# shuwang127/SRCNN_Cpp

Measured on AMD Instinct MI355X. Metric: SRCNN Y-channel Mpixels/sec, higher is better.
Workload: dtype f32; 1 GPU; 1 x 3840x2160 luma plane per GPU per step (1920x1080 x2.0, BASELINE configs[1]), fused conv path, mfma arithmetic, inputs resident in HBM; frames_per_gpu=1, width=3840, height=2160, mode=mfma, seam_deferral=True, output_checksum=584152

## Files before the change

srcnn_cpp_amd/csrc/srcnn_kernels.h:

```cpp
#pragma once
#include <hip/hip_runtime.h>
#include <stddef.h>
#include <stdint.h>

namespace srcnn {

constexpr int FW = 128;
constexpr int YP = FW + 8;
constexpr int YR = 16;
constexpr int NWAVES = FW / 32;
constexpr int NTHREADS = NWAVES * 64;

enum StripMode { MODE_FUSED = 0, MODE_L12 = 1, MODE_L3 = 2 };

constexpr int NFRAG_L1 = 82;
constexpr int NFRAG_L2 = 32;
constexpr int NFRAG_L3 = 16;
constexpr int NFRAG_B2 = 16;
constexpr int NFRAG_L2U = 32;
constexpr int NFRAG_B2U = 16;
constexpr int NFRAG_L3U = 16;
constexpr int FRAG_L2 = NFRAG_L1, FRAG_L3 = FRAG_L2 + NFRAG_L2, FRAG_B2 = FRAG_L3 + NFRAG_L3,
              FRAG_L2U = FRAG_B2 + NFRAG_B2, FRAG_B2U = FRAG_L2U + NFRAG_L2U, FRAG_L3U = FRAG_B2U + NFRAG_B2U;
constexpr int NFRAG = FRAG_L3U + NFRAG_L3U;

__host__ __device__ constexpr int acc_row(int r, int h) { return (r & 3) + 8 * (r >> 2) + 4 * h; }
__host__ __device__ constexpr int row_chan(int i) { return 2 * ((i & 3) + 4 * (i >> 3)) + ((i >> 2) & 1); }

__host__ __device__ constexpr int l3_row_tap(int i)
{
    const int r = (i & 3) + 4 * (i >> 3), h = (i >> 2) & 1, s = r / 5, m = r % 5, n = h ? 3 + s : s;
    return (r < 15 && n < 5) ? 5 * m + n : -1;
}
__host__ __device__ constexpr bool l3_row_is_scale(int i)
{
    const int r = (i & 3) + 4 * (i >> 3), h = (i >> 2) & 1;
    return h == 1 && r >= 10 && r < 15;
}

constexpr int S16_FRAG_L2 = 24, S16_FRAG_L3 = 32, S16_NFRAG = 36;
constexpr size_t S16_TABLE_BYTES = (size_t)S16_NFRAG * 64 * 16 + 2 * 16 * sizeof(float);
__host__ __device__ constexpr int l1s_tap(int b, int h, int e)
{
    const int n = 4 * b + e / 2, u = e & 1;
    if (n < 20) return (2 * (n % 5) + u < 9) ? 9 * (n / 5 + 5 * h) + 2 * (n % 5) + u : -1;
    if (n < 23) {
        const int jj = 4 * h + 2 * (n - 20) + u;
        return (h == 0 ? jj <= 3 : (jj >= 4 && jj <= 8)) ? 36 + jj : -1;
    }
    return (u == 0 && h == 0) ? 81 : -1;
}

struct StripParams {
    const uint8_t *src;
    long src_stride, src_frame_pitch;
    int src_row0;
    const uint8_t *src_top, *src_bot;
    long halo_stride;
    int src_row1;
    const float *planes_in;
    float *planes_out;
    long pl_stride, pl_pitch, pl_frame_pitch;
    uint8_t *dst;
    float *pre;
    long dst_stride, dst_frame_pitch;
    int dst_row0;
    const float *wfrag;
    const uint32_t *wfrag16;
    float *sink;
    float b3;
    int width, height;
    int row_begin, row_end;
    int seg_rows, n_strips, n_segs;
    const int *items;
    int items_per_frame;
    int seams_per_frame;
    float *seam;
    float *cseam;
    int strips_total;
    int tune;
    uint8_t *flag;
    float fix_delta, fix_scale;
    float fix_kl, fix_abs;
    unsigned *fix_counters;
};

enum { FIX_N_SCAT = 0, FIX_N_DENSE = 1, FIX_N_CHANGED = 2, FIX_MAX_DEV = 3, FIX_N_RERUN = 4,
       FIX_MAX_RATIO = 5,
       FIX_TOTALS = 6,
       FIX_WORD_STRIDE = 64,
       FIX_NEXT_ITEM = 6,
       FIX_NEXT_RERUN = 7,
       FIX_REGIONS = 8, FIX_REGION0 = 8 * FIX_WORD_STRIDE,
       FIX_COUNTERS = FIX_REGION0 + FIX_REGIONS * FIX_WORD_STRIDE };
struct FixParams {
    const uint8_t *src;
    long src_stride;
    int src_row0;
    const uint8_t *src_top, *src_bot;
    long halo_stride;
    int src_row1;
    uint8_t *dst;
    const uint8_t *flag;
    long dst_stride;
    int dst_row0;
    int width, height, row_begin, row_end;
    const float *wraw;
    unsigned *counters;
    unsigned long long *totals;
    unsigned *scat, *dense;
// ... 106 lines not shown
```

srcnn_cpp_amd/csrc/srcnn_mfma.hip:

```cpp
#include "srcnn_kernels.h"

#include <type_traits>

#ifndef SRCNN_SAFE_HAZARDS
#define SRCNN_SAFE_HAZARDS 0
#endif
#if SRCNN_SAFE_HAZARDS
#define SRCNN_KNS safe
#else
#define SRCNN_KNS fast
#endif

namespace srcnn {
namespace SRCNN_KNS {

typedef float f32x16 __attribute__((ext_vector_type(16)));
typedef float f32x2 __attribute__((ext_vector_type(2)));

#define MFMA(a, b, c) __builtin_amdgcn_mfma_f32_32x32x2f32((a), (b), (c), 0, 0, 0)

__device__ __forceinline__ f32x16 mfma_first(float a, float b, const f32x16 &c)
{
#if SRCNN_SAFE_HAZARDS
    return MFMA(a, b, c);
#endif
    f32x16 d;
    asm volatile("v_mfma_f32_32x32x2_f32 %0, %1, %2, %3" : "=&v"(d) : "v"(a), "v"(b), "v"(c));
    return d;
}
__device__ __forceinline__ f32x16 mfma_first0(float a, float b)
{
#if SRCNN_SAFE_HAZARDS
    const f32x16 z = {0};
    return MFMA(a, b, z);
#endif
    f32x16 d;
    asm volatile("v_mfma_f32_32x32x2_f32 %0, %1, %2, 0" : "=&v"(d) : "v"(a), "v"(b));
    return d;
}


__device__ __forceinline__ int clampi(int v, int lo, int hi) { return min(max(v, lo), hi); }

__device__ __forceinline__ unsigned lane_off(unsigned x)
{
    asm volatile("" : "+v"(x));
    return x;
}
template <typename T>
__device__ __forceinline__ __attribute__((address_space(1))) T *scalar_base(T *p)
{
    __attribute__((address_space(1))) T *g = (__attribute__((address_space(1))) T *)p;
    asm volatile("" : "+s"(g));
    return g;
}

template <typename T>
__device__ __forceinline__ T *uniform_ptr(T *p)
{
    const unsigned long long a = (unsigned long long)p;
    const unsigned lo = __builtin_amdgcn_readfirstlane((unsigned)a), hi = __builtin_amdgcn_readfirstlane((unsigned)(a >> 32));
    return (T *)(((unsigned long long)hi << 32) | lo);
}

__device__ __forceinline__ void lds_barrier()
{
    asm volatile("s_waitcnt lgkmcnt(0)\n\ts_barrier" ::: "memory");
}

__device__ __forceinline__ float relu(float x)
{
    float r;
    asm("v_max_f32 %0, 0, %1" : "=v"(r) : "v"(x));
    return r;
}

__device__ const signed char CSEAM_TERMS[15][9] = {
    {4, 0, 124, 1, 125, 2, 126, 3, 127}, {3, 0, 125, 1, 126, 2, 127, 0, 0}, {1, 0, 126, 0, 0, 0, 0, 0, 0},
    {1, 0, 127, 0, 0, 0, 0, 0, 0},       {1, 1, 127, 0, 0, 0, 0, 0, 0},     {1, 2, 0, 0, 0, 0, 0, 0, 0},
    {1, 3, 1, 0, 0, 0, 0, 0, 0},         {1, 4, 2, 0, 0, 0, 0, 0, 0},       {1, 1, 0, 0, 0, 0, 0, 0, 0},
    {1, 2, 1, 0, 0, 0, 0, 0, 0},         {1, 3, 2, 0, 0, 0, 0, 0, 0},       {1, 4, 3, 0, 0, 0, 0, 0, 0},
    {1, 3, 0, 0, 0, 0, 0, 0, 0},         {1, 4, 0, 0, 0, 0, 0, 0, 0},       {1, 4, 1, 0, 0, 0, 0, 0, 0}};

struct CseamLane {
    int cnt, off[4];
};
__device__ __forceinline__ CseamLane cseam_lane(int e)
{
    CseamLane cl = {0, {0, 0, 0, 0}};
    if (e < 15) {
        const signed char *t = CSEAM_TERMS[e];
        cl.cnt = t[0];
#pragma unroll
        for (int i = 0; i < 4; ++i) cl.off[i] = i < t[0] ? t[1 + 2 * i] * FW + t[2 + 2 * i] : 0;
    }
    return cl;
}
__device__ __forceinline__ void cseam_export(const float *tile, float *dst, int e, const CseamLane &cl)
{
    const float a = tile[cl.off[0]], b = tile[cl.off[1]], c = tile[cl.off[2]], d = tile[cl.off[3]];
    float v = a;
    v = cl.cnt > 1 ? v + b : v;
    v = cl.cnt > 2 ? v + c : v;
    v = cl.cnt > 3 ? v + d : v;
    if (cl.cnt > 0) dst[(unsigned)e] = v;
}

__device__ __forceinline__ void relu_pairs(f32x16 &a, const f32x2 ones)
{
#if SRCNN_SAFE_HAZARDS
#pragma unroll
    for (int q = 0; q < 16; ++q) a[q] = __builtin_fmaxf(a[q], 0.f);
    return;
#endif
#pragma unroll
    for (int q = 0; q < 8; ++q) {
        f32x2 pr = {a[2 * q], a[2 * q + 1]};
        asm("v_pk_mul_f32 %0, %0, %1 clamp" : "+v"(pr) : "s"(ones));
        a[2 * q] = pr.x;
        a[2 * q + 1] = pr.y;
    }
}

constexpr bool fast_kernel(int mode, bool pre, int diag)
{
    (void)diag;
    return mode == MODE_FUSED && !pre;
}

template <int MODE, bool PRE, int DIAG = 0, bool FIX = false, bool HALO3 = false>
__device__ __forceinline__ void strip_body(const StripParams &p)
{
    static_assert(!FIX || (MODE == MODE_FUSED && !PRE && DIAG == 0), "flags belong to the production fused kernel");
    static_assert(!HALO3 || (MODE == MODE_FUSED && !PRE && DIAG == 0), "halo buffers belong to the production fused kernel");
    if constexpr (FIX) {
        if (blockIdx.x == 0)
            for (int i = threadIdx.x; i < FIX_COUNTERS; i += 256) p.fix_counters[i] = 0u;
    }
    unsigned long long lt[4] = {0, 0, 0, 0};
    if constexpr (DIAG == 2) lt[0] = __builtin_amdgcn_s_memrealtime();
    extern __shared__ __attribute__((aligned(16))) char smem[];
    float *ylds = reinterpret_cast<float *>(smem);
    float *fbuf = (MODE == MODE_L3) ? ylds : ylds + 2 * YR * YP;

    const int tid = threadIdx.x;
    const int lane = tid & 63;
    const int wave = __builtin_amdgcn_readfirstlane(tid >> 6);
    const int j = lane & 31;
    const int half = lane >> 5;

    constexpr int HALO = (MODE == MODE_L12) ? 0 : 2;

    const int W = p.width, H = p.height;
    int bid = blockIdx.x;
    int strip, frame = 0, ys, ye, seam_up = -1, seam_dn = -1;
    if (p.items) {
        frame = bid / p.items_per_frame;
        const int *it = p.items + ITEM_INTS * (bid - frame * p.items_per_frame);
        strip = it[0];
        ys = it[1];
        ye = it[2];
        if constexpr (MODE == MODE_FUSED) {
            seam_up = it[3] >= 0 ? it[3] + frame * p.seams_per_frame : -1;
            seam_dn = it[4] >= 0 ? it[4] + frame * p.seams_per_frame : -1;
        }
        if (ys >= ye) return;
    } else {
        if (!(p.tune & 8)) {
            const int nwg = gridDim.x, q = nwg >> 3, r = nwg & 7, xcd = bid & 7;
            bid = (xcd < r ? xcd * (q + 1) : r * (q + 1) + (xcd - r) * q) + (bid >> 3);
        }
        strip = bid % p.n_strips;
        bid /= p.n_strips;
        const int seg = bid % p.n_segs;
        frame = bid / p.n_segs;
        ys = p.row_begin + seg * p.seg_rows;
        ye = min(ys + p.seg_rows, p.row_end);
    }

    const bool cs = (MODE != MODE_L12) && p.cseam != nullptr;
    const CseamLane cl = cseam_lane((cs && threadIdx.x < 64 && (threadIdx.x & 31) < 15 &&
                                     (threadIdx.x < 32 || fast_kernel(MODE, PRE, DIAG)))
                                        ? (int)(threadIdx.x & 31) : 15);
    const int halo_c = cs ? 0 : HALO;
    const int xs = strip * (FW - 2 * halo_c);
    const int gx0 = xs - halo_c;
    float *cs_row0 = (cs && wave == 0)
                         ? p.cseam + (((long)frame * p.strips_total + strip) * (p.row_end - p.row_begin) - p.row_begin) * CSEAM_FLOATS
                         : nullptr;
    const bool top_open = seam_up >= 0, bot_open = seam_dn >= 0;
    const int f_lo = top_open ? ys : max(ys - HALO, 0);
    const int f_hi = bot_open ? ye : min(ye + HALO, H);
    const int out_lo = top_open ? ys + 2 : ys, out_hi = bot_open ? ye - 2 : ye;

    const float *wf = p.wfrag + lane;
    float w1f[2][41], w2f[32], w3f[16];
    f32x16 b2v = {0};
    if constexpr (MODE != MODE_L3) {
#pragma unroll
        for (int t = 0; t < 2; ++t)
#pragma unroll
            for (int s = 0; s < 41; ++s) w1f[t][s] = wf[(t * 41 + s) * 64];
        constexpr int L2 = (MODE == MODE_L12) ? FRAG_L2U : FRAG_L2, B2 = (MODE == MODE_L12) ? FRAG_B2U : FRAG_B2;
#pragma unroll
        for (int q = 0; q < 32; ++q) w2f[q] = wf[(L2 + q) * 64];
#pragma unroll
        for (int q = 0; q < 16; ++q) b2v[q] = wf[(B2 + q) * 64];
    }
    if constexpr (MODE != MODE_L12) {
        constexpr int L3 = (MODE == MODE_L3) ? FRAG_L3U : FRAG_L3;
#pragma unroll
        for (int q = 0; q < 16; ++q) w3f[q] = wf[(L3 + q) * 64];
    }
    const f32x2 ones = {1.0f, 1.0f};

    const uint8_t *srcf = nullptr;
    int ycol = 0;
    if constexpr (MODE != MODE_L3) {
        srcf = p.src + (long)frame * p.src_frame_pitch;
        ycol = clampi(gx0 - 4 + tid, 0, W - 1);
    }
    const int y_last = min(H - 1, f_hi + 3);
    auto y_row = [&](int r) -> const uint8_t * {
        if constexpr (HALO3) {
            if (r < p.src_row0) return p.src_top + (long)(r - (p.src_row0 - 6)) * p.halo_stride;
            if (r >= p.src_row1) return p.src_bot + (long)(r - p.src_row1) * p.halo_stride;
        }
        return srcf + (long)(r - p.src_row0) * p.src_stride;
    };
    auto load_y = [&](int r) -> uint8_t {
        const uint8_t *row = y_row(clampi(r, 0, y_last));
        return row[(unsigned)ycol];
    };
    auto stage_y = [&](int r, uint8_t v) {
        const int slot = r & (YR - 1);
        const float fv = (float)v;
        ylds[slot * YP + tid] = fv;
        ylds[(slot + YR) * YP + tid] = fv;
    };
    if constexpr (MODE != MODE_L3) {
        if (tid < YP) {
            uint8_t v[9];
#pragma unroll
            for (int q = 0; q < 9; ++q) v[q] = load_y(f_lo - 4 + q);
#pragma unroll
            for (int q = 0; q < 9; ++q) stage_y(f_lo - 4 + q, v[q]);
        }
        __syncthreads();
    }
    asm volatile("s_waitcnt vmcnt(0)" ::: "memory");
    if constexpr (MODE != MODE_L3) {
#pragma unroll
        for (int t = 0; t < 2; ++t)
#pragma unroll
            for (int k = 0; k < 41; ++k) asm volatile("" : "+v"(w1f[t][k]));
#pragma unroll
        for (int q = 0; q < 32; ++q) asm volatile("" : "+v"(w2f[q]));
        asm volatile("" : "+v"(b2v));
    }
    if constexpr (MODE != MODE_L12) {
#pragma unroll
        for (int q = 0; q < 16; ++q) asm volatile("" : "+v"(w3f[q]));
    }

    if constexpr (DIAG == 2) lt[1] = __builtin_amdgcn_s_memrealtime();

    const int xi = 32 * wave + j;
    const int gx = gx0 + xi;


    constexpr bool FASTK = fast_kernel(MODE, PRE, DIAG);
    static_assert(!FIX || FASTK, "the flag threshold reads plane 5 through the FAST kernels' column offsets");
    constexpr int FSLOT = 6 * FW;
    int xn[5] = {0, 0, 0, 0, 0};
    bool px_ok = false;
    if constexpr (MODE != MODE_L12) {
#pragma unroll
        for (int n = 0; n < 5; ++n) {
            xn[n] = clampi(clampi(gx + n - 2, 0, W - 1) - gx0, 0, FW - 1);
            if constexpr (FASTK) xn[n] += n * FW + half * FSLOT;
        }
        px_ok = cs ? (gx < W) && (xi >= 2 || strip == 0) && (xi < FW - 2 || strip == p.strips_total - 1)
                   : (xi >= HALO) && (xi < FW - HALO) && (gx < W);
    }
    CseamLane cl2 = cl;
    if constexpr (FASTK) {
#pragma unroll
        for (int i = 0; i < 4; ++i) cl2.off[i] += half * FSLOT;
    }
    float R[4][3] = {{0.f, 0.f, 0.f}, {0.f, 0.f, 0.f}, {0.f, 0.f, 0.f}, {0.f, 0.f, 0.f}};
    long o_out = (long)frame * p.dst_frame_pitch + (long)(f_lo - 3 - p.dst_row0) * p.dst_stride;
    long o_src = (long)(min(f_lo + 5, y_last) - p.src_row0) * p.src_stride;
    long o_pl = (long)frame * p.pl_frame_pitch + (long)(MODE == MODE_L3 ? min(f_lo + 1, H - 1) : f_lo) * p.pl_stride;
    auto scale_thr = [&](const float *fr) -> float {
        float s1 = fr[xn[0] + 5 * FW];
#pragma unroll
        for (int n = 1; n < 5; ++n) s1 += fr[xn[n] + (5 - n) * FW];
        return fix_threshold(s1, p.fix_delta, p.fix_kl, p.fix_abs);
    };
    auto finalize = [&](long o, float acc, bool ok, const float *fr) {
        const float v = acc + p.b3;
        auto row = scalar_base(p.dst + o);
        if (ok) row[lane_off((unsigned)gx)] = (uint8_t)clampi((int)v, 0, 255);
        if constexpr (FIX) {
            auto frow = scalar_base(p.flag + o);
            const float thr = scale_thr(fr);
            if (ok) frow[lane_off((unsigned)gx)] = fix_code(v, thr, p.fix_delta, p.fix_scale);
        }
        if constexpr (PRE) {
            float *prow = p.pre + o;
            if (ok) prow[(unsigned)gx] = v;
        }
    };
    auto ftile = [&](int g, int slot) -> float * {
        if constexpr (FASTK) return fbuf + ((4 - ((g + slot) & 3)) & 3) * FSLOT;
        else return fbuf + (((g & 1) * 3 + slot) * 6) * FW;
    };
    auto vertical = [&](int f, const f32x16 &t) {
        const int fplane = 3 * half * FW + xi;
        if (top_open && f < ys + SEAM_ROWS) {
            const int r = f - ys;
            float *o = p.seam + ((long)seam_up * SEAM_FLOATS + seam_t_off(r)) * NTHREADS + tid;
#pragma unroll
            for (int s = 0; s < 3; ++s)
#pragma unroll
                for (int m = 1; m < 5; ++m)
                    if (m > r) o[(s * (4 - r) + (m - r - 1)) * NTHREADS] = t[5 * s + m];
        }
        if (f > 0) {
            float *fo = ftile(f, 0) + fplane;
#pragma unroll
            for (int s = 0; s < 3; ++s) {
                fo[s * FW] = R[3][s] + t[5 * s + 4];
                R[3][s] = R[2][s] + t[5 * s + 3];
                R[2][s] = R[1][s] + t[5 * s + 2];
                R[1][s] = R[0][s] + t[5 * s + 1];
                R[0][s] = t[5 * s];
            }
        } else {
#pragma unroll
            for (int s = 0; s < 3; ++s) {
                R[0][s] = t[5 * s];
                R[1][s] = t[5 * s] + t[5 * s + 1];
                R[2][s] = R[1][s] + t[5 * s + 2];
                R[3][s] = 0.f;
            }
        }
        if (f == H - 1) {
            float *f1 = ftile(f, 1) + fplane, *f2 = ftile(f, 2) + fplane;
#pragma unroll
            for (int s = 0; s < 3; ++s) {
                f1[s * FW] = R[3][s] + t[5 * s + 4];
                f2[s * FW] = (R[2][s] + t[5 * s + 3]) + t[5 * s + 4];
            }
        }
    };
    float hv[5];
    auto hp_load = [&](int g, int slot) {
        const float *fr = ftile(g, slot);
#pragma unroll
        for (int n = 0; n < 5; ++n) hv[n] = FASTK ? fr[xn[n]] : fr[n * FW + xn[n]];
    };
    auto hp_use = [&](int g, int slot) {
        float acc = hv[0];
#pragma unroll
        for (int n = 1; n < 5; ++n) acc += hv[n];
        const int y = g - 2 + slot;
        const bool rows_ok = (y >= out_lo) && (y < out_hi) && (!FASTK || half == 0);
        finalize(slot == 0 ? o_out : o_out + (long)slot * p.dst_stride, acc, px_ok && rows_ok, ftile(g, slot));
        if (cs_row0 && rows_ok) cseam_export(ftile(g, slot), cs_row0 + y * CSEAM_FLOATS, lane, FASTK ? cl2 : cl);
    };
    const unsigned st2 = (unsigned)gx + (half ? 0u : (unsigned)p.dst_stride);
    const unsigned cs2 = (unsigned)(lane & 31) + (half ? 0u : (unsigned)CSEAM_FLOATS);
    const int do_cs = __builtin_amdgcn_readfirstlane((cs && wave == 0) ? 1 : 0);
    auto hp2_load = [&](int slot) {
        const float *fr = fbuf + slot * FSLOT;
#pragma unroll
        for (int n = 0; n < 5; ++n) hv[n] = fr[xn[n]];
    };
    float v2 = 0.f;
    auto hp2_use = [&](int f, int slot) {
        float acc = hv[0];
#pragma unroll
        for (int n = 1; n < 5; ++n) acc += hv[n];
        const float v = acc + p.b3;
        auto row = scalar_base(p.dst + (o_out - p.dst_stride));
        if (px_ok) row[lane_off(st2)] = (uint8_t)clampi((int)v, 0, 255);
        if constexpr (FIX) {
            v2 = v;
            const float *fr = fbuf + slot * FSLOT;
#pragma unroll
            for (int n = 0; n < 5; ++n) hv[n] = fr[xn[n] + (5 - n) * FW];
        }
        if (do_cs) {
            const float *tile = fbuf + slot * FSLOT;
            const float a = tile[cl2.off[0]], b = tile[cl2.off[1]], c = tile[cl2.off[2]], d = tile[cl2.off[3]];
            float e = a;
            e = cl2.cnt > 1 ? e + b : e;
            e = cl2.cnt > 2 ? e + c : e;
            e = cl2.cnt > 3 ? e + d : e;
            auto dst = scalar_base(cs_row0 + (f - 4) * CSEAM_FLOATS);
            if (cl2.cnt > 0) dst[cs2] = e;
        }
    };

    auto hp2_flag = [&]() {
        float s1 = hv[0];
#pragma unroll
        for (int n = 1; n < 5; ++n) s1 += hv[n];
        const float thr = fix_threshold(s1, p.fix_delta, p.fix_kl, p.fix_abs);
        auto frow = scalar_base(p.flag + (o_out - p.dst_stride));
        if (px_ok) frow[lane_off(st2)] = fix_code(v2, thr, p.fix_delta, p.fix_scale);
    };

    f32x16 d2n = {0};
    const unsigned pl_lane = (MODE == MODE_L12) ? (unsigned)(half * p.pl_pitch + gx)
                                                : (unsigned)(half * p.pl_pitch + clampi(gx, 0, W - 1));
    auto load_planes_at = [&](long o) {
        const float *q = p.planes_in + o;
        const unsigned lo = lane_off(pl_lane * 4u);
#pragma unroll
        for (int r = 0; r < 16; ++r)
            d2n[r] = __builtin_nontemporal_load((const __attribute__((address_space(1))) float *)((const __attribute__((address_space(1))) char *)scalar_base(q + (long)(2 * r) * p.pl_pitch) + lo));
    };
    if constexpr (MODE == MODE_L3) load_planes_at((long)frame * p.pl_frame_pitch + (long)f_lo * p.pl_stride);
    auto drain = [&](int g) {
        const int nslots = (g == H - 1) ? 3 : 1;
        for (int slot = 0; slot < nslots; ++slot) {
            hp_load(g, slot);
            hp_use(g, slot);
        }
    };
    auto row = [&](int f, auto ph_tag) {
        constexpr int PH = decltype(ph_tag)::value;
        constexpr bool FAST = PH >= 0;
        const int g = f - 1;
        const bool hp = FAST ? (PH & 1) != 0 : (MODE != MODE_L12) && (g >= f_lo);
        constexpr int SLOT_W = (4 - PH) & 3;
        constexpr int SLOT_R = (4 - ((PH + 3) & 3)) & 3;

        f32x16 d2;
        if constexpr (MODE != MODE_L3) {
            unsigned ynext;
            asm volatile("" : "=v"(ynext));
            if constexpr (HALO3) {
                const uint8_t *yr = uniform_ptr(y_row(min(f + 5, y_last)));
                if (tid < YP) ynext = scalar_base(yr)[lane_off((unsigned)ycol)];
            } else {
                if (tid < YP) ynext = scalar_base(srcf + o_src)[lane_off((unsigned)ycol)];
                if (f + 5 < y_last) o_src += p.src_stride;
            }

            const float *yb = ylds + ((f - 4) & (YR - 1)) * YP + xi;
            const float *ybN = yb + half;
            const float *ybW = yb + (half ? YP - 8 : 0);
            auto ldb = [&](int s) -> float {
                const int ki = (2 * s) / 9, kj = (2 * s) % 9;
                if (s == 40) return half ? 1.0f : yb[8 * YP + 8];
                if (kj == 8) return ybW[ki * YP + kj];
                return ybN[ki * YP + kj];
            };
            f32x16 a0 = {0}, a1 = {0};
            auto layer1 = [&](auto with_pb) {
                constexpr bool PB = decltype(with_pb)::value;
                constexpr int PF = 3;
                float bq[41];
#pragma unroll
                for (int s = 0; s < PF; ++s) bq[s] = ldb(s);
#pragma unroll
                for (int s = 0; s < 41; ++s) {
                    if (s + PF < 41) bq[s + PF] = ldb(s + PF);
                    if constexpr (PB && MODE != MODE_L12) {
                        if constexpr (FAST) {
                            if (s == 2) hp2_load(SLOT_R);
                            if (s == 8) hp2_use(f, SLOT_R);
                            if constexpr (FIX) {
                                if (s == 14) hp2_flag();
                            }
                        } else {
                            if (s == 2) hp_load(g, 0);
                            if (s == 8) hp_use(g, 0);
                        }
                    }
                    a0 = MFMA(w1f[0][s], bq[s], a0);
                    a1 = MFMA(w1f[1][s], bq[s], a1);
                    __builtin_amdgcn_sched_barrier(0);
                }
            };
            if constexpr (FAST) {
                layer1(std::integral_constant<bool, (PH & 1) != 0>{});
            } else {
                if (hp) layer1(std::true_type{});
                else layer1(std::false_type{});
            }
            relu_pairs(a0, ones);
            relu_pairs(a1, ones);
            __builtin_amdgcn_sched_barrier(0);

            d2 = mfma_first(w2f[0], a0[0], b2v);
#pragma unroll
            for (int r = 1; r < 16; ++r) d2 = MFMA(w2f[r], a0[r], d2);
#pragma unroll
            for (int r = 0; r < 16; ++r) d2 = MFMA(w2f[16 + r], a1[r], d2);
            __builtin_amdgcn_sched_barrier(0);
            if constexpr (MODE == MODE_L12) {
#pragma unroll
                for (int r = 0; r < 16; ++r) d2[r] = relu(d2[r]);
            } else {
                relu_pairs(d2, ones);
            }
            __builtin_amdgcn_sched_barrier(0);

            asm volatile("" : "+v"(ynext));
            if (tid < YP) stage_y(f + 5, (uint8_t)ynext);

            if constexpr (MODE == MODE_L12) {
                if (gx < W) {
                    float *o = p.planes_out + o_pl;
                    const unsigned lo = lane_off(pl_lane * 4u);
#pragma unroll
                    for (int r = 0; r < 16; ++r)
                        __builtin_nontemporal_store(d2[r], (__attribute__((address_space(1))) float *)((__attribute__((address_space(1))) char *)scalar_base(o + (long)(2 * r) * p.pl_pitch) + lo));
                }
            }
        } else {
            d2 = d2n;
            load_planes_at(o_pl);
            if constexpr (FAST) {
                if constexpr ((PH & 1) != 0) {
                    hp2_load(SLOT_R);
                    hp2_use(f, SLOT_R);
                }
            } else if (hp) {
                hp_load(g, 0);
                hp_use(g, 0);
            }
        }

        if constexpr (MODE != MODE_L12) {
            f32x16 t = {0};
            if constexpr (MODE == MODE_FUSED) {
                t = mfma_first0(w3f[0], d2[0]);
#pragma unroll
                for (int r = 1; r < 16; ++r) t = MFMA(w3f[r], d2[r], t);
            } else {
#pragma unroll
                for (int r = 0; r < 16; ++r) t = MFMA(w3f[r], d2[r], t);
            }
            __builtin_amdgcn_sched_barrier(0);
            if constexpr (FAST) {
                float *fo = fbuf + SLOT_W * FSLOT + 3 * half * FW + xi;
#pragma unroll
                for (int s = 0; s < 3; ++s) {
                    fo[s * FW] = R[3][s] + t[5 * s + 4];
#ifndef SRCNN_ABL_NO_CHAIN_ADDS
                    R[3][s] = R[2][s] + t[5 * s + 3];
                    R[2][s] = R[1][s] + t[5 * s + 2];
                    R[1][s] = R[0][s] + t[5 * s + 1];
                    R[0][s] = t[5 * s];
#endif
                    asm volatile("" : "+v"(R[0][s]), "+v"(R[1][s]), "+v"(R[2][s]), "+v"(R[3][s]));
                }
            } else {
                vertical(f, t);
            }
        }

        if constexpr (FASTK) __builtin_amdgcn_sched_barrier(0);
        lds_barrier();
        if constexpr (FASTK) __builtin_amdgcn_sched_barrier(0);
        o_out += p.dst_stride;
        if constexpr (MODE == MODE_L3) {
            if (f + 1 < H - 1) o_pl += p.pl_stride;
        } else {
            o_pl += p.pl_stride;
        }
    };
    {
        int f = f_lo;
        if constexpr (FASTK) {
            const int f_a = (f_lo + 6 + 1) & ~1;
            const int f_b = min(f_hi, H - 1) & ~1;
            for (; f < f_hi && f < f_a; ++f) row(f, std::integral_constant<int, -1>{});
            if ((f & 2) && f + 2 <= f_b) {
                row(f, std::integral_constant<int, 2>{});
                row(f + 1, std::integral_constant<int, 3>{});
// ... 177 lines not shown
    if (winmap && (winmap[(long)v * rows + yrel] | winmap[(long)(v + 1) * rows + yrel])) return;
    const float *es = p.cseam + (((long)frame * p.strips_total + v) * rows + yrel) * CSEAM_FLOATS;
    const float *et = es + (long)rows * CSEAM_FLOATS;
    cseam_pixels<PRE, FIX>(p, es, et, frame, p.row_begin + yrel, (v + 1) * FW);
}

template <bool PRE, bool FIX>
__global__ __launch_bounds__(256) void srcnn_cseam_kernel(const StripParams p)
{
    cseam_block<PRE, FIX>(p, (long)blockIdx.x, (int)blockIdx.y, nullptr);
}

template <bool PRE, bool FIX>
__global__ __launch_bounds__(NTHREADS) void srcnn_seams_merged_kernel(const StripParams p, const int *__restrict__ seams, int n_seams,
                                                                     const unsigned char *__restrict__ winmap, int cblocks_per_frame)
{
    static_assert(NTHREADS == 256, "both roles use 256 threads");
    if ((int)blockIdx.x < n_seams) {
        seam_block<PRE, true, FIX>(p, seams, (int)blockIdx.x);
    } else {
        const int q = (int)blockIdx.x - n_seams;
        cseam_block<PRE, FIX>(p, (long)(q % cblocks_per_frame), q / cblocks_per_frame, winmap);
    }
}

size_t strip_lds_bytes(int mode);

template <bool HALO3>
__global__ __launch_bounds__(NTHREADS, 2) void srcnn_strip_fold_kernel(const StripParams p, const FoldParams f)
{
    if ((int)blockIdx.x >= f.first_block) {
        const int q = (int)blockIdx.x - f.first_block;
        if (q >= f.n_seams) cseam_block<false, false>(f.prev, (long)(q - f.n_seams), 0, f.winmap);
        else if (f.winmap) seam_block<false, true, false>(f.prev, f.seams, q);
        else seam_block<false, false, false>(f.prev, f.seams, q);
        return;
    }
    fast::strip_body<MODE_FUSED, false, 0, false, HALO3>(p);
}

hipError_t launch_strip_fold(const StripParams &p, const FoldParams &f, hipStream_t stream, size_t lds_pad)
{
    if (p.pre || p.flag || f.prev.pre || f.prev.flag || !p.items) return hipErrorInvalidValue;
    const dim3 grid((unsigned)(f.first_block + f.n_seams + f.cblocks)), block(NTHREADS);
    const size_t lds = strip_lds_bytes(MODE_FUSED) + lds_pad;
    if (p.src_top || p.src_bot) hipLaunchKernelGGL((srcnn_strip_fold_kernel<true>), grid, block, lds, stream, p, f);
    else hipLaunchKernelGGL((srcnn_strip_fold_kernel<false>), grid, block, lds, stream, p, f);
    return hipGetLastError();
}

hipError_t launch_cseams(const StripParams &p, int n_frames, hipStream_t stream)
{
    const long n = (long)(p.strips_total - 1) * (p.row_end - p.row_begin);
    if (n <= 0) return hipSuccess;
    const dim3 grid((unsigned)((n + 255) / 256), (unsigned)n_frames);
    if (p.flag) hipLaunchKernelGGL((srcnn_cseam_kernel<false, true>), grid, dim3(256), 0, stream, p);
    else if (p.pre) hipLaunchKernelGGL((srcnn_cseam_kernel<true, false>), grid, dim3(256), 0, stream, p);
    else hipLaunchKernelGGL((srcnn_cseam_kernel<false, false>), grid, dim3(256), 0, stream, p);
    return hipGetLastError();
}

hipError_t launch_seams_merged(const StripParams &p, int n_seams , const int *d_seams, const unsigned char *d_winmap,
                               int n_frames, hipStream_t stream)
{
    const long n = (long)(p.strips_total - 1) * (p.row_end - p.row_begin);
    const int cb = (int)((n + 255) / 256);
    const dim3 grid((unsigned)(n_seams + cb * n_frames));
    if (p.flag) hipLaunchKernelGGL((srcnn_seams_merged_kernel<false, true>), grid, dim3(NTHREADS), 0, stream, p, d_seams, n_seams, d_winmap, cb);
    else if (p.pre) hipLaunchKernelGGL((srcnn_seams_merged_kernel<true, false>), grid, dim3(NTHREADS), 0, stream, p, d_seams, n_seams, d_winmap, cb);
    else hipLaunchKernelGGL((srcnn_seams_merged_kernel<false, false>), grid, dim3(NTHREADS), 0, stream, p, d_seams, n_seams, d_winmap, cb);
    return hipGetLastError();
}

hipError_t launch_seams(const StripParams &p, int n_seams , const int *d_seams, hipStream_t stream)
{
    if (p.flag) hipLaunchKernelGGL((srcnn_seam_kernel<false, true>), dim3(n_seams), dim3(NTHREADS), 0, stream, p, d_seams);
    else if (p.pre) hipLaunchKernelGGL((srcnn_seam_kernel<true, false>), dim3(n_seams), dim3(NTHREADS), 0, stream, p, d_seams);
    else hipLaunchKernelGGL((srcnn_seam_kernel<false, false>), dim3(n_seams), dim3(NTHREADS), 0, stream, p, d_seams);
    return hipGetLastError();
}

size_t strip_lds_bytes(int mode)
{
    return sizeof(float) * ((mode == MODE_L3 ? 0 : 2 * YR * YP) + 2 * 3 * 6 * FW);
}

#endif

#if SRCNN_SAFE_HAZARDS
#define launch_strip launch_strip_safe
static size_t strip_lds_bytes_safe(int mode) { return sizeof(float) * ((mode == MODE_L3 ? 0 : 2 * YR * YP) + 2 * 3 * 6 * FW); }
#define strip_lds_bytes strip_lds_bytes_safe
#endif

hipError_t launch_strip(int mode, const StripParams &p, int n_frames, hipStream_t stream, size_t lds_pad)
{
    const dim3 grid((unsigned)((long)p.n_strips * p.n_segs * n_frames));
    const dim3 block(NTHREADS);
    const size_t lds = strip_lds_bytes(mode) + lds_pad;
    const bool pre = p.pre != nullptr;
    switch (mode) {
    case MODE_FUSED:
        if (p.src_top || p.src_bot) {
            if (pre || (p.tune & 16) || n_frames != 1) return hipErrorInvalidValue;
            if (p.flag) hipLaunchKernelGGL((srcnn_strip_kernel<MODE_FUSED, false, 0, true, true>), grid, block, lds, stream, p);
            else hipLaunchKernelGGL((srcnn_strip_kernel<MODE_FUSED, false, 0, false, true>), grid, block, lds, stream, p);
        }
        else if (p.flag) {
            if (pre) return hipErrorInvalidValue;
            hipLaunchKernelGGL((srcnn_strip_kernel<MODE_FUSED, false, 0, true>), grid, block, lds, stream, p);
        }
        else if (p.tune & 16) hipLaunchKernelGGL((srcnn_strip_kernel<MODE_FUSED, false, 2>), grid, block, lds, stream, p);
        else if (pre) hipLaunchKernelGGL((srcnn_strip_kernel<MODE_FUSED, true>), grid, block, lds, stream, p);
        else hipLaunchKernelGGL((srcnn_strip_kernel<MODE_FUSED, false>), grid, block, lds, stream, p);
        break;
    case MODE_L12:
        hipLaunchKernelGGL((srcnn_strip_kernel<MODE_L12, false>), grid, block, lds, stream, p);
        break;
    case MODE_L3:
        if (pre) hipLaunchKernelGGL((srcnn_strip_kernel<MODE_L3, true>), grid, block, lds, stream, p);
        else hipLaunchKernelGGL((srcnn_strip_kernel<MODE_L3, false>), grid, block, lds, stream, p);
        break;
    default: return hipErrorInvalidValue;
    }
    return hipGetLastError();
}

}
```

srcnn_cpp_amd/csrc/srcnn_model.cpp:

```cpp
#include "srcnn_ctx.h"

using namespace srcnn;
using namespace srcnn::host;

namespace srcnn {
namespace host {

int scale_exponent(double bound)
{
    if (!(bound > 0.0) || !std::isfinite(bound)) return 0;
    int e = 0;
    (void)std::frexp(bound * (1.0 + 1.0 / 65536.0), &e);
    return e;
}

float fixup_delta(const float *w1, const float *b1, const float *w2, const float *b2, const float *w3, double margin)
{
    double a1[64], m2 = 0.0, s3 = 0.0;
    for (int c = 0; c < 64; ++c) {
        double s = 0.0;
        for (int t = 0; t < 81; ++t) s += std::max(w1[c * 81 + t], 0.f);
        a1[c] = std::max(0.0, 255.0 * s + b1[c]);
    }
    for (int k = 0; k < 32; ++k) {
        double s = b2[k];
        for (int i = 0; i < 64; ++i) s += (double)std::max(w2[k * 64 + i], 0.f) * a1[i];
        m2 = std::max(m2, s);
    }
    for (int i = 0; i < 800; ++i) s3 += (double)w3[i] * w3[i];
    const double d = margin * std::ldexp(1.0, -24) * std::sqrt(s3) * m2 + 4.0 * std::ldexp(1.0, -24) * 256.0;
    if (!std::isfinite(d)) return 0.25f;
    return (float)std::min(0.25, std::max(d, 1e-6));
}

void layer_scales(const float *w1, const float *b1, const float *w2, const float *b2, int *e1, int *e2)
{
    double a1[64], m1 = 0.0, m2 = 0.0;
    for (int c = 0; c < 64; ++c) {
        double s = 0.0;
        for (int t = 0; t < 81; ++t) s += std::max(w1[c * 81 + t], 0.f);
        a1[c] = std::max(0.0, 255.0 * s + b1[c]);
        m1 = std::max(m1, a1[c]);
    }
    for (int k = 0; k < 32; ++k) {
        double s = b2[k];
        for (int i = 0; i < 64; ++i) s += (double)std::max(w2[k * 64 + i], 0.f) * a1[i];
        m2 = std::max(m2, s);
    }
    *e1 = scale_exponent(m1);
    *e2 = scale_exponent(m2);
}

void pack_fragments(const float *w1 , const float *b1, const float *w2 ,
                    const float *b2, const float *w3 , float *out )
{
    int e1, e2;
    layer_scales(w1, b1, w2, b2, &e1, &e2);
    for (int l = 0; l < 64; ++l) {
        const int i = l & 31, kk = l >> 5;
        const int ch = row_chan(i);
        for (int t = 0; t < 2; ++t)
            for (int s = 0; s < 41; ++s) {
                const int tap = 2 * s + kk, c = 32 * t + ch;
                out[(t * 41 + s) * 64 + l] = std::ldexp(tap < 81 ? w1[c * 81 + tap] : b1[c], -e1);
            }
        for (int t = 0; t < 2; ++t)
            for (int r = 0; r < 16; ++r) {
                const float w = w2[ch * 64 + 32 * t + 2 * r + kk];
                out[(FRAG_L2 + t * 16 + r) * 64 + l] = std::ldexp(w, e1 - e2);
                out[(FRAG_L2U + t * 16 + r) * 64 + l] = std::ldexp(w, e1);
            }
        for (int r = 0; r < 16; ++r) {
            const int tap = l3_row_tap(i);
            const float w = tap >= 0 ? w3[(2 * r + kk) * 25 + tap] : 0.f;
            float a = 0.f;
            if (l3_row_is_scale(i))
                for (int t = 0; t < 25; ++t) a = std::max(a, std::fabs(w3[(2 * r + kk) * 25 + t]));
            out[(FRAG_L3 + r) * 64 + l] = std::ldexp(tap >= 0 ? w : a, e2);
            out[(FRAG_L3U + r) * 64 + l] = w;
        }
        for (int r = 0; r < 16; ++r) {
            out[(FRAG_B2 + r) * 64 + l] = std::ldexp(b2[2 * r + kk], -e2);
            out[(FRAG_B2U + r) * 64 + l] = b2[2 * r + kk];
        }
    }
}

void split16(float w, float scale, uint16_t *hi, uint16_t *lo)
{
    const float ws = w * scale;
    const _Float16 h = (_Float16)ws;
    const _Float16 l = (_Float16)(ws - (float)h);
    std::memcpy(hi, &h, 2);
    std::memcpy(lo, &l, 2);
}

void pack_fragments16(const float *w1 , const float *b1, const float *w2 ,
                      const float *b2, const float *w3 , uint8_t *out )
{
    constexpr float SCALE = 16384.f, SCALE1 = 2048.f;
    uint16_t *tab = reinterpret_cast<uint16_t *>(out);
    auto slot = [&](int frag, int l, int e) -> uint16_t * { return tab + ((size_t)frag * 64 + l) * 8 + e; };
    for (int l = 0; l < 64; ++l) {
        const int m = l & 31, h = l >> 5;
        for (int e = 0; e < 8; ++e) {
            for (int t = 0; t < 2; ++t)
                for (int b = 0; b < 6; ++b) {
                    const int tap = l1s_tap(b, h, e), c = 32 * t + m;
                    const float w = tap < 0 ? 0.f : (tap == 81 ? b1[c] : w1[c * 81 + tap]);
                    split16(w, tap == 81 ? 0.125f : SCALE1, slot((2 * t) * 6 + b, l, e), slot((2 * t + 1) * 6 + b, l, e));
                }
            for (int b = 0; b < 4; ++b) {
                const int c1 = 32 * (b >> 1) + acc_row(8 * (b & 1) + e, h);
                split16(w2[m * 64 + c1], SCALE, slot(S16_FRAG_L2 + b, l, e), slot(S16_FRAG_L2 + 4 + b, l, e));
            }
            for (int b = 0; b < 2; ++b) {
                const int c2 = acc_row(8 * b + e, h), tap = l3_row_tap(m);
                float a = 0.f;
                if (l3_row_is_scale(m))
                    for (int t = 0; t < 25; ++t) a = std::max(a, std::fabs(w3[c2 * 25 + t]));
                split16(tap >= 0 ? w3[c2 * 25 + tap] : a, SCALE, slot(S16_FRAG_L3 + b, l, e),
                        slot(S16_FRAG_L3 + 2 + b, l, e));
            }
        }
    }
    float *b2t = reinterpret_cast<float *>(out + (size_t)S16_NFRAG * 64 * 16);
    for (int h = 0; h < 2; ++h)
        for (int r = 0; r < 16; ++r) b2t[h * 16 + r] = b2[acc_row(r, h)] * 0.0625f;
}

bool split16_range_ok(const float *w1, const float *b1, const float *w2, const float *b2, const float *w3)
{
    float a1[64], wmax1 = 0.f, wmax23 = 0.f, a1max = 0.f, a2max = 0.f;
    for (int c = 0; c < 64; ++c) {
        double s = 0;
        for (int t = 0; t < 81; ++t) {
            s += std::max(w1[c * 81 + t], 0.f);
            wmax1 = std::max(wmax1, std::fabs(w1[c * 81 + t]));
        }
        a1[c] = std::max(0.f, (float)(255.0 * s + b1[c]));
        a1max = std::max(a1max, a1[c]);
        wmax1 = std::max(wmax1, std::fabs(b1[c]) / 256.f);
    }
    for (int k = 0; k < 32; ++k) {
        double s = b2[k];
        for (int i = 0; i < 64; ++i) {
            s += (double)std::max(w2[k * 64 + i], 0.f) * a1[i];
            wmax23 = std::max(wmax23, std::fabs(w2[k * 64 + i]));
// ... 141 lines not shown
```

srcnn_cpp_amd/csrc/srcnn_probe.hip:

```cpp
#include "srcnn_kernels.h"

#include <vector>

namespace srcnn {

typedef float f32x16 __attribute__((ext_vector_type(16)));
typedef float f32x2 __attribute__((ext_vector_type(2)));
#define PROBE_WAIT() do { if constexpr (WAIT) asm volatile("s_nop 15\n\ts_nop 15" ::: "memory"); } while (0)

template <bool WAIT>
__global__ __launch_bounds__(256) void interlock_probe_kernel(const float *__restrict__ in, float *__restrict__ out, int iters)
{
    const int t = blockIdx.x * blockDim.x + threadIdx.x;
    float a = in[t], b = in[t + 4096], w = in[t + 2048] * 0.25f, r = 0.f;
    const f32x2 ones = {1.0f, 1.0f};
    f32x16 cinit;
    for (int q = 0; q < 16; ++q) cinit[q] = in[(t + 64 * q) & 4095] * 0.125f;
    for (int k = 0; k < iters; ++k) {
        f32x16 acc, acc2, acc3;
        asm volatile("v_mfma_f32_32x32x2_f32 %0, %1, %2, 0" : "=&v"(acc) : "v"(a), "v"(b));
        PROBE_WAIT();
#pragma unroll
        for (int q = 0; q < 8; ++q) {
            f32x2 pr = {acc[2 * q], acc[2 * q + 1]};
            asm volatile("v_pk_mul_f32 %0, %0, %1 clamp" : "+v"(pr) : "s"(ones));
            acc[2 * q] = pr.x;
            acc[2 * q + 1] = pr.y;
        }
        PROBE_WAIT();
        asm volatile("v_mfma_f32_32x32x2_f32 %0, %1, %2, %3" : "=&v"(acc2) : "v"(w), "v"(acc[0]), "v"(cinit));
        PROBE_WAIT();
#pragma unroll
        for (int q = 1; q < 16; ++q) acc2 = __builtin_amdgcn_mfma_f32_32x32x2f32(w, acc[q], acc2, 0, 0, 0);
        PROBE_WAIT();
#pragma unroll
        for (int q = 0; q < 8; ++q) {
            f32x2 pr = {acc2[2 * q], acc2[2 * q + 1]};
            asm volatile("v_pk_mul_f32 %0, %0, %1 clamp" : "+v"(pr) : "s"(ones));
            acc2[2 * q] = pr.x;
            acc2[2 * q + 1] = pr.y;
        }
        PROBE_WAIT();
        asm volatile("v_mfma_f32_32x32x2_f32 %0, %1, %2, 0" : "=&v"(acc3) : "v"(w), "v"(acc2[0]));
        PROBE_WAIT();
#pragma unroll
        for (int q = 1; q < 16; ++q) acc3 = __builtin_amdgcn_mfma_f32_32x32x2f32(w, acc2[q], acc3, 0, 0, 0);
        float s = 0.f;
#pragma unroll
        for (int q = 0; q < 16; ++q) s += acc3[q] + acc2[q] * 0.5f + acc[q] * 0.25f;
        r = r * 0.5f + s;
        a = a * 0.5f + 0.25f * w;
        b = b * 0.75f + 0.1f;
    }
    out[t] = r;
}

long interlock_probe_mismatches(int device, hipStream_t st)
{
    constexpr int kThreads = 256, kBlocks = 512, n = kThreads * kBlocks;
    int prev = -1;
    if (hipGetDevice(&prev) != hipSuccess) prev = -1;
    if (hipSetDevice(device) != hipSuccess) return -1;
    std::vector<float> h((size_t)n + 4096);
    for (size_t i = 0; i < h.size(); ++i) h[i] = (float)((i * 2654435761u) % 1000) / 250.f - 2.f;
    float *d_in = nullptr, *d_a = nullptr, *d_b = nullptr;
    long bad = -1;
    if (hipMalloc(&d_in, h.size() * 4) == hipSuccess && hipMalloc(&d_a, (size_t)n * 4) == hipSuccess &&
        hipMalloc(&d_b, (size_t)n * 4) == hipSuccess &&
        hipMemcpyAsync(d_in, h.data(), h.size() * 4, hipMemcpyHostToDevice, st) == hipSuccess) {
        bad = 0;
        std::vector<float> ra((size_t)n), rb((size_t)n);
        for (int rep = 0; rep < 2 && bad >= 0; ++rep) {
            hipLaunchKernelGGL(interlock_probe_kernel<false>, dim3(kBlocks), dim3(kThreads), 0, st, d_in, d_a, 24);
            hipLaunchKernelGGL(interlock_probe_kernel<true>, dim3(kBlocks), dim3(kThreads), 0, st, d_in, d_b, 24);
            if (hipGetLastError() != hipSuccess || hipMemcpyAsync(ra.data(), d_a, (size_t)n * 4, hipMemcpyDeviceToHost, st) != hipSuccess ||
                hipMemcpyAsync(rb.data(), d_b, (size_t)n * 4, hipMemcpyDeviceToHost, st) != hipSuccess ||
                hipStreamSynchronize(st) != hipSuccess) {
                bad = -1;
                break;
            }
            long nonzero = 0;
            for (int i = 0; i < n; ++i) {
                bad += ra[(size_t)i] != rb[(size_t)i];
                nonzero += rb[(size_t)i] != 0.f;
            }
            if (nonzero < n / 2) bad += n;
        }
    }
    (void)hipStreamSynchronize(st);
    if (d_in) (void)hipFree(d_in);
    if (d_a) (void)hipFree(d_a);
    if (d_b) (void)hipFree(d_b);
    if (prev >= 0 && prev != device) (void)hipSetDevice(prev);
    return bad;
}

}
```

Measured before the change: 8811 MPix/s.

## Move layer-1/2 biases and layer-3 weights to LDS, fold last tap into 32x32x1 MFMA

The layer-1 bias and last tap are no longer folded into a 41st 32x32x2 MFMA step using a constant-1 input. The last tap is now applied with one 32x32x1 MFMA over a combined 32-wide accumulator, and the bias is added together with ReLU via clamped packed adds. Layer-2 bias and layer-3 weights move from per-lane registers into LDS and are reloaded each row, which frees VGPRs. The cost is extra LDS traffic and a larger LDS footprint, and the interlock probe is extended to check the new instruction pattern.

Result: no change. 8841 MPix/s, median of 6 (+0.3%).

```diff
diff --git a/srcnn_cpp_amd/csrc/srcnn_kernels.h b/srcnn_cpp_amd/csrc/srcnn_kernels.h
--- a/srcnn_cpp_amd/csrc/srcnn_kernels.h
+++ b/srcnn_cpp_amd/csrc/srcnn_kernels.h
@@ -14,6 +14,8 @@
 enum StripMode { MODE_FUSED = 0, MODE_L12 = 1, MODE_L3 = 2 };
 
 constexpr int NFRAG_L1 = 82;
+constexpr int FRAG_L1T = 40;
+constexpr int FRAG_B1 = 81;
 constexpr int NFRAG_L2 = 32;
 constexpr int NFRAG_L3 = 16;
 constexpr int NFRAG_B2 = 16;
@@ -26,6 +28,8 @@
 
 __host__ __device__ constexpr int acc_row(int r, int h) { return (r & 3) + 8 * (r >> 2) + 4 * h; }
 __host__ __device__ constexpr int row_chan(int i) { return 2 * ((i & 3) + 4 * (i >> 3)) + ((i >> 2) & 1); }
+
+__host__ __device__ constexpr int bias_table_chan(int e) { return 32 * ((e >> 4) & 1) + 2 * (e & 15) + (e >> 5); }
 
 __host__ __device__ constexpr int l3_row_tap(int i)
 {
diff --git a/srcnn_cpp_amd/csrc/srcnn_mfma.hip b/srcnn_cpp_amd/csrc/srcnn_mfma.hip
--- a/srcnn_cpp_amd/csrc/srcnn_mfma.hip
+++ b/srcnn_cpp_amd/csrc/srcnn_mfma.hip
@@ -14,19 +14,21 @@
 namespace srcnn {
 namespace SRCNN_KNS {
 
+typedef float f32x32 __attribute__((ext_vector_type(32)));
 typedef float f32x16 __attribute__((ext_vector_type(16)));
+typedef float f32x4 __attribute__((ext_vector_type(4)));
 typedef float f32x2 __attribute__((ext_vector_type(2)));
 
 #define MFMA(a, b, c) __builtin_amdgcn_mfma_f32_32x32x2f32((a), (b), (c), 0, 0, 0)
-
-__device__ __forceinline__ f32x16 mfma_first(float a, float b, const f32x16 &c)
+#define MFMA2B(a, b, c) __builtin_amdgcn_mfma_f32_32x32x1f32((a), (b), (c), 0, 0, 0)
+
+__device__ __forceinline__ void mfma_first_inplace(float a, float b, f32x16 &c)
 {
 #if SRCNN_SAFE_HAZARDS
-    return MFMA(a, b, c);
+    c = MFMA(a, b, c);
+    return;
 #endif
-    f32x16 d;
-    asm volatile("v_mfma_f32_32x32x2_f32 %0, %1, %2, %3" : "=&v"(d) : "v"(a), "v"(b), "v"(c));
-    return d;
+    asm volatile("v_mfma_f32_32x32x2_f32 %0, %1, %2, %0" : "+v"(c) : "v"(a), "v"(b));
 }
 __device__ __forceinline__ f32x16 mfma_first0(float a, float b)
 {
@@ -122,6 +124,33 @@
     }
 }
 
+template <int BLOCK>
+__device__ __forceinline__ void bias_relu_pairs(f32x32 &a, const f32x16 &bv)
+{
+#if SRCNN_SAFE_HAZARDS
+#pragma unroll
+    for (int q = 0; q < 16; ++q) a[16 * BLOCK + q] = __builtin_fmaxf(a[16 * BLOCK + q] + bv[q], 0.f);
+    return;
+#endif
+#pragma unroll
+    for (int q = 0; q < 8; ++q) {
+        f32x2 pr = {a[16 * BLOCK + 2 * q], a[16 * BLOCK + 2 * q + 1]};
+        const f32x2 bp = {bv[2 * q], bv[2 * q + 1]};
+        asm("v_pk_add_f32 %0, %0, %1 clamp" : "+v"(pr) : "v"(bp));
+        a[16 * BLOCK + 2 * q] = pr.x;
+        a[16 * BLOCK + 2 * q + 1] = pr.y;
+    }
+}
+typedef const __attribute__((address_space(3))) float *lds_cfloat_ptr;
+__device__ __forceinline__ void lds_read16(f32x16 &v, lds_cfloat_ptr p)
+{
+#pragma unroll
+    for (int q = 0; q < 4; ++q) {
+        const f32x4 b = reinterpret_cast<const __attribute__((address_space(3))) f32x4 *>(p)[q];
+        v[4 * q] = b.x, v[4 * q + 1] = b.y, v[4 * q + 2] = b.z, v[4 * q + 3] = b.w;
+    }
+}
+
 constexpr bool fast_kernel(int mode, bool pre, int diag)
 {
     (void)diag;
@@ -142,6 +171,8 @@
     extern __shared__ __attribute__((aligned(16))) char smem[];
     float *ylds = reinterpret_cast<float *>(smem);
     float *fbuf = (MODE == MODE_L3) ? ylds : ylds + 2 * YR * YP;
+    float *blds = fbuf + 2 * 3 * 6 * FW;
+    float *w3lds = blds + 128;
 
     const int tid = threadIdx.x;
     const int lane = tid & 63;
@@ -194,20 +225,19 @@
     const int out_lo = top_open ? ys + 2 : ys, out_hi = bot_open ? ye - 2 : ye;
 
     const float *wf = p.wfrag + lane;
-    float w1f[2][41], w2f[32], w3f[16];
-    f32x16 b2v = {0};
+    float w1f[2][40], w1t = 0.f, w2f[32], w3f[16];
     if constexpr (MODE != MODE_L3) {
 #pragma unroll
         for (int t = 0; t < 2; ++t)
 #pragma unroll
-            for (int s = 0; s < 41; ++s) w1f[t][s] = wf[(t * 41 + s) * 64];
-        constexpr int L2 = (MODE == MODE_L12) ? FRAG_L2U : FRAG_L2, B2 = (MODE == MODE_L12) ? FRAG_B2U : FRAG_B2;
+            for (int s = 0; s < 40; ++s) w1f[t][s] = wf[(t * 41 + s) * 64];
+        w1t = wf[FRAG_L1T * 64];
+        constexpr int L2 = (MODE == MODE_L12) ? FRAG_L2U : FRAG_L2;
 #pragma unroll
         for (int q = 0; q < 32; ++q) w2f[q] = wf[(L2 + q) * 64];
-#pragma unroll
-        for (int q = 0; q < 16; ++q) b2v[q] = wf[(B2 + q) * 64];
-    }
-    if constexpr (MODE != MODE_L12) {
+    }
+    constexpr bool W3_LDS = MODE == MODE_FUSED;
+    if constexpr (MODE != MODE_L12 && !W3_LDS) {
         constexpr int L3 = (MODE == MODE_L3) ? FRAG_L3U : FRAG_L3;
 #pragma unroll
         for (int q = 0; q < 16; ++q) w3f[q] = wf[(L3 + q) * 64];
@@ -246,6 +276,13 @@
 #pragma unroll
             for (int q = 0; q < 9; ++q) stage_y(f_lo - 4 + q, v[q]);
         }
+        constexpr int B2 = (MODE == MODE_L12) ? FRAG_B2U : FRAG_B2;
+        if (tid < 64) blds[tid] = p.wfrag[FRAG_B1 * 64 + tid];
+        else if (tid < 128 && (tid & 16) == 0) blds[tid] = p.wfrag[(B2 + (tid & 15)) * 64 + (tid & 32)];
+        if constexpr (W3_LDS) {
+#pragma unroll
+            for (int k = 0; k < 4; ++k) w3lds[256 * k + tid] = p.wfrag[(FRAG_L3 + 4 * k + (tid & 3)) * 64 + (tid >> 2)];
+        }
         __syncthreads();
     }
     asm volatile("s_waitcnt vmcnt(0)" ::: "memory");
@@ -253,12 +290,12 @@
 #pragma unroll
         for (int t = 0; t < 2; ++t)
 #pragma unroll
-            for (int k = 0; k < 41; ++k) asm volatile("" : "+v"(w1f[t][k]));
+            for (int k = 0; k < 40; ++k) asm volatile("" : "+v"(w1f[t][k]));
+        asm volatile("" : "+v"(w1t));
 #pragma unroll
         for (int q = 0; q < 32; ++q) asm volatile("" : "+v"(w2f[q]));
-        asm volatile("" : "+v"(b2v));
-    }
-    if constexpr (MODE != MODE_L12) {
+    }
+    if constexpr (MODE != MODE_L12 && !W3_LDS) {
 #pragma unroll
         for (int q = 0; q < 16; ++q) asm volatile("" : "+v"(w3f[q]));
     }
@@ -414,6 +451,8 @@
     };
 
     f32x16 d2n = {0};
+    lds_cfloat_ptr bias_lds = (lds_cfloat_ptr)(blds + 32 * half);
+    lds_cfloat_ptr w3_lds = (lds_cfloat_ptr)(w3lds + 4 * lane);
     const unsigned pl_lane = (MODE == MODE_L12) ? (unsigned)(half * p.pl_pitch + gx)
                                                 : (unsigned)(half * p.pl_pitch + clampi(gx, 0, W - 1));
     auto load_planes_at = [&](long o) {
@@ -456,11 +495,12 @@
             const float *ybW = yb + (half ? YP - 8 : 0);
             auto ldb = [&](int s) -> float {
                 const int ki = (2 * s) / 9, kj = (2 * s) % 9;
-                if (s == 40) return half ? 1.0f : yb[8 * YP + 8];
+                if (s == 40) return yb[8 * YP + 8];
                 if (kj == 8) return ybW[ki * YP + kj];
                 return ybN[ki * YP + kj];
             };
             f32x16 a0 = {0}, a1 = {0};
+            float b80 = 0.f;
             auto layer1 = [&](auto with_pb) {
                 constexpr bool PB = decltype(with_pb)::value;
                 constexpr int PF = 3;
@@ -468,7 +508,7 @@
 #pragma unroll
                 for (int s = 0; s < PF; ++s) bq[s] = ldb(s);
 #pragma unroll
-                for (int s = 0; s < 41; ++s) {
+                for (int s = 0; s < 40; ++s) {
                     if (s + PF < 41) bq[s + PF] = ldb(s + PF);
                     if constexpr (PB && MODE != MODE_L12) {
                         if constexpr (FAST) {
@@ -484,8 +524,10 @@
                     }
                     a0 = MFMA(w1f[0][s], bq[s], a0);
                     a1 = MFMA(w1f[1][s], bq[s], a1);
+                    asm volatile("" : "+v"(a0), "+v"(a1));
                     __builtin_amdgcn_sched_barrier(0);
                 }
+                b80 = bq[40];
             };
             if constexpr (FAST) {
                 layer1(std::integral_constant<bool, (PH & 1) != 0>{});
@@ -493,15 +535,35 @@
                 if (hp) layer1(std::true_type{});
                 else layer1(std::false_type{});
             }
-            relu_pairs(a0, ones);
-            relu_pairs(a1, ones);
+            asm volatile("" : "+v"(bias_lds));
+            f32x16 bvb;
+            lds_read16(d2, bias_lds);
+            lds_read16(bvb, bias_lds + 16);
             __builtin_amdgcn_sched_barrier(0);
-
-            d2 = mfma_first(w2f[0], a0[0], b2v);
-#pragma unroll
-            for (int r = 1; r < 16; ++r) d2 = MFMA(w2f[r], a0[r], d2);
-#pragma unroll
-            for (int r = 0; r < 16; ++r) d2 = MFMA(w2f[16 + r], a1[r], d2);
+            f32x32 a01 = __builtin_shufflevector(a0, a1, 0, 1, 2, 3, 4, 5, 6, 7, 8, 9, 10, 11, 12, 13, 14, 15, 16, 17, 18, 19, 20, 21, 22,
+                                                 23, 24, 25, 26, 27, 28, 29, 30, 31);
+            a01 = MFMA2B(w1t, b80, a01);
+            __builtin_amdgcn_sched_barrier(0);
+            bias_relu_pairs<0>(a01, d2);
+            __builtin_amdgcn_sched_barrier(0);
+            lds_read16(d2, bias_lds + 64);
+            __builtin_amdgcn_sched_barrier(0);
+            bias_relu_pairs<1>(a01, bvb);
+            __builtin_amdgcn_sched_barrier(0);
+
+            mfma_first_inplace(w2f[0], a01[0], d2);
+            if constexpr (W3_LDS) {
+                __builtin_amdgcn_sched_barrier(0);
+                asm volatile("" : "+v"(w3_lds));
+#pragma unroll
+                for (int q = 0; q < 4; ++q) {
+                    const f32x4 b = reinterpret_cast<const __attribute__((address_space(3))) f32x4 *>(w3_lds + 256 * q)[0];
+                    w3f[4 * q] = b.x, w3f[4 * q + 1] = b.y, w3f[4 * q + 2] = b.z, w3f[4 * q + 3] = b.w;
+                }
+                __builtin_amdgcn_sched_barrier(0);
+            }
+#pragma unroll
+            for (int r = 1; r < 32; ++r) d2 = MFMA(w2f[r], a01[r], d2);
             __builtin_amdgcn_sched_barrier(0);
             if constexpr (MODE == MODE_L12) {
 #pragma unroll
@@ -845,14 +907,14 @@
 
 size_t strip_lds_bytes(int mode)
 {
-    return sizeof(float) * ((mode == MODE_L3 ? 0 : 2 * YR * YP) + 2 * 3 * 6 * FW);
+    return sizeof(float) * ((mode == MODE_L3 ? 0 : 2 * YR * YP + 128 + 1024) + 2 * 3 * 6 * FW);
 }
 
 #endif
 
 #if SRCNN_SAFE_HAZARDS
 #define launch_strip launch_strip_safe
-static size_t strip_lds_bytes_safe(int mode) { return sizeof(float) * ((mode == MODE_L3 ? 0 : 2 * YR * YP) + 2 * 3 * 6 * FW); }
+static size_t strip_lds_bytes_safe(int mode) { return sizeof(float) * ((mode == MODE_L3 ? 0 : 2 * YR * YP + 128 + 1024) + 2 * 3 * 6 * FW); }
 #define strip_lds_bytes strip_lds_bytes_safe
 #endif
 
diff --git a/srcnn_cpp_amd/csrc/srcnn_model.cpp b/srcnn_cpp_amd/csrc/srcnn_model.cpp
--- a/srcnn_cpp_amd/csrc/srcnn_model.cpp
+++ b/srcnn_cpp_amd/csrc/srcnn_model.cpp
@@ -60,10 +60,12 @@
         const int i = l & 31, kk = l >> 5;
         const int ch = row_chan(i);
         for (int t = 0; t < 2; ++t)
-            for (int s = 0; s < 41; ++s) {
+            for (int s = 0; s < 40; ++s) {
                 const int tap = 2 * s + kk, c = 32 * t + ch;
-                out[(t * 41 + s) * 64 + l] = std::ldexp(tap < 81 ? w1[c * 81 + tap] : b1[c], -e1);
-            }
+                out[(t * 41 + s) * 64 + l] = std::ldexp(w1[c * 81 + tap], -e1);
+            }
+        out[FRAG_L1T * 64 + l] = std::ldexp(w1[(32 * kk + ch) * 81 + 80], -e1);
+        out[FRAG_B1 * 64 + l] = std::ldexp(b1[bias_table_chan(l)], -e1);
         for (int t = 0; t < 2; ++t)
             for (int r = 0; r < 16; ++r) {
                 const float w = w2[ch * 64 + 32 * t + 2 * r + kk];
diff --git a/srcnn_cpp_amd/csrc/srcnn_probe.hip b/srcnn_cpp_amd/csrc/srcnn_probe.hip
--- a/srcnn_cpp_amd/csrc/srcnn_probe.hip
+++ b/srcnn_cpp_amd/csrc/srcnn_probe.hip
@@ -4,6 +4,7 @@
 
 namespace srcnn {
 
+typedef float f32x32 __attribute__((ext_vector_type(32)));
 typedef float f32x16 __attribute__((ext_vector_type(16)));
 typedef float f32x2 __attribute__((ext_vector_type(2)));
 #define PROBE_WAIT() do { if constexpr (WAIT) asm volatile("s_nop 15\n\ts_nop 15" ::: "memory"); } while (0)
@@ -55,6 +56,45 @@
     out[t] = r;
 }
 
+template <bool WAIT>
+__global__ __launch_bounds__(256) void interlock_probe2_kernel(const float *__restrict__ in, float *__restrict__ out, int iters)
+{
+    const int t = blockIdx.x * blockDim.x + threadIdx.x;
+    float a = in[t], b = in[t + 4096], w = in[t + 2048] * 0.25f, r = 0.f;
+    f32x16 cinit;
+    for (int q = 0; q < 16; ++q) cinit[q] = in[(t + 64 * q) & 4095] * 0.125f;
+    f32x2 bias[16];
+    for (int q = 0; q < 16; ++q) bias[q] = f32x2{in[(t + 128 * q + 1) & 4095], in[(t + 128 * q + 65) & 4095]} * 0.25f;
+    for (int k = 0; k < iters; ++k) {
+        const f32x16 z = {0};
+        const f32x16 c0 = __builtin_amdgcn_mfma_f32_32x32x2f32(a, b, z, 0, 0, 0), c1 = __builtin_amdgcn_mfma_f32_32x32x2f32(w, b, z, 0, 0, 0);
+        f32x32 acc = __builtin_shufflevector(c0, c1, 0, 1, 2, 3, 4, 5, 6, 7, 8, 9, 10, 11, 12, 13, 14, 15, 16, 17, 18, 19, 20, 21, 22, 23, 24,
+                                             25, 26, 27, 28, 29, 30, 31);
+        acc = __builtin_amdgcn_mfma_f32_32x32x1f32(w, a, acc, 0, 0, 0);
+        PROBE_WAIT();
+#pragma unroll
+        for (int q = 0; q < 16; ++q) {
+            f32x2 pr = {acc[2 * q], acc[2 * q + 1]};
+            asm volatile("v_pk_add_f32 %0, %0, %1 clamp" : "+v"(pr) : "v"(bias[q]));
+            acc[2 * q] = pr.x;
+            acc[2 * q + 1] = pr.y;
+        }
+        PROBE_WAIT();
+        f32x16 acc2 = cinit;
+        asm volatile("v_mfma_f32_32x32x2_f32 %0, %1, %2, %0" : "+v"(acc2) : "v"(w), "v"(acc[0]));
+        PROBE_WAIT();
+#pragma unroll
+        for (int q = 1; q < 32; ++q) acc2 = __builtin_amdgcn_mfma_f32_32x32x2f32(w, acc[q], acc2, 0, 0, 0);
+        float s = 0.f;
+#pragma unroll
+        for (int q = 0; q < 16; ++q) s += acc2[q] + acc[q] * 0.5f + acc[16 + q] * 0.25f;
+        r = r * 0.5f + s;
+        a = a * 0.5f + 0.25f * w;
+        b = b * 0.75f + 0.1f;
+    }
+    out[t] = r;
+}
+
 long interlock_probe_mismatches(int device, hipStream_t st)
 {
     constexpr int kThreads = 256, kBlocks = 512, n = kThreads * kBlocks;
@@ -70,9 +110,14 @@
         hipMemcpyAsync(d_in, h.data(), h.size() * 4, hipMemcpyHostToDevice, st) == hipSuccess) {
         bad = 0;
         std::vector<float> ra((size_t)n), rb((size_t)n);
-        for (int rep = 0; rep < 2 && bad >= 0; ++rep) {
-            hipLaunchKernelGGL(interlock_probe_kernel<false>, dim3(kBlocks), dim3(kThreads), 0, st, d_in, d_a, 24);
-            hipLaunchKernelGGL(interlock_probe_kernel<true>, dim3(kBlocks), dim3(kThreads), 0, st, d_in, d_b, 24);
+        for (int rep = 0; rep < 4 && bad >= 0; ++rep) {
+            if (rep & 1) {
+                hipLaunchKernelGGL(interlock_probe2_kernel<false>, dim3(kBlocks), dim3(kThreads), 0, st, d_in, d_a, 24);
+                hipLaunchKernelGGL(interlock_probe2_kernel<true>, dim3(kBlocks), dim3(kThreads), 0, st, d_in, d_b, 24);
+            } else {
+                hipLaunchKernelGGL(interlock_probe_kernel<false>, dim3(kBlocks), dim3(kThreads), 0, st, d_in, d_a, 24);
+                hipLaunchKernelGGL(interlock_probe_kernel<true>, dim3(kBlocks), dim3(kThreads), 0, st, d_in, d_b, 24);
+            }
             if (hipGetLastError() != hipSuccess || hipMemcpyAsync(ra.data(), d_a, (size_t)n * 4, hipMemcpyDeviceToHost, st) != hipSuccess ||
                 hipMemcpyAsync(rb.data(), d_b, (size_t)n * 4, hipMemcpyDeviceToHost, st) != hipSuccess ||
                 hipStreamSynchronize(st) != hipSuccess) {
```
